# yangao07/abPOA

Measured on NVIDIA B200. Metric: GCUPS (DP cells/s), global/convex 10 kbp, higher is better.
Workload: dtype int16 (packed int16x2 DPX arithmetic; int32 kernel only as overflow fallback)

## Files before the change

abpoa_b200/csrc/poa_kernels.cu:

```cuda
#include <cuda_runtime.h>
#include <stdint.h>
#include <algorithm>
#include "poa_device.cuh"
#include "poa_chain.cuh"

#define FULL 0xffffffffu
#define NEG POA_NEG32

enum { LG = 0, AG = 1, CG = 2 };
enum { GLOBAL = 0, LOCAL = 1, EXTEND = 2 };

#define OP_M   0x1
#define OP_E1  0x2
#define OP_E2  0x4
#define OP_E   0x6
#define OP_F1  0x8
#define OP_F2  0x10
#define OP_F   0x18
#define OP_ALL 0x1f

__device__ __forceinline__ void ld8(const int16_t *p, int v[8]) {
    const uint4 u = *reinterpret_cast<const uint4 *>(p);
    v[0] = (int)(short)(u.x & 0xffff); v[1] = ((int)u.x) >> 16;
    v[2] = (int)(short)(u.y & 0xffff); v[3] = ((int)u.y) >> 16;
// ... 815 lines not shown
        c.KF1[k] = pk_host(-(oe1 + e1 * (2 * k - 1)), -(oe1 + e1 * (2 * k))); c.KF2[k] = pk_host(-(oe2 + e2 * (2 * k - 1)), -(oe2 + e2 * (2 * k)));
        c.KLG[k] = pk_host(-e1 * (2 * k), -e1 * (2 * k + 1));
    }
    c.NE1 = pk_host(-e1, -e1); c.NOE1 = pk_host(-oe1, -oe1); c.NE2 = pk_host(-e2, -e2); c.NOE2 = pk_host(-oe2, -oe2);
    return c;
}

struct P16Smem {
    int *mat_s; uint4 *cap_lo, *cap_hi, *ring_meta; int16_t *ring_data;
};
__device__ __forceinline__ P16Smem p16_smem_init(uint8_t *dyn_smem, const PoaParamsDev *prm, int ring_rows, int lane) {
    P16Smem sm;
    sm.mat_s = reinterpret_cast<int *>(dyn_smem);
    sm.cap_lo = reinterpret_cast<uint4 *>(dyn_smem + POA_MAX_M * POA_MAX_M * sizeof(int));
    sm.cap_hi = sm.cap_lo + 9;
    sm.ring_meta = sm.cap_hi + 9;
    sm.ring_data = reinterpret_cast<int16_t *>(sm.ring_meta + ring_rows);
    const int m = prm->m;
    for (int t = lane; t < m * m; t += 32) sm.mat_s[t] = prm->mat[t];
    if (lane < 9) {
        unsigned lo[4], hi[4];
#pragma unroll
        for (int k = 0; k < 4; ++k) {
            lo[k] = pk(2 * k < lane ? NEGP : 32767, 2 * k + 1 < lane ? NEGP : 32767);
            hi[k] = pk(2 * k >= 8 - lane ? NEGP : 32767, 2 * k + 1 >= 8 - lane ? NEGP : 32767);
        }
        sm.cap_lo[lane] = make_uint4(lo[0], lo[1], lo[2], lo[3]);
        sm.cap_hi[lane] = make_uint4(hi[0], hi[1], hi[2], hi[3]);
    }
    __syncwarp();
    return sm;
}

template <int GAP, int MODE, bool LEAN = false, bool TMA = false>
__device__ __forceinline__ void p16_run_job(const PoaJobDesc &jd, const PoaParamsDev *__restrict__ prm, const P16Consts &kc, const P16Smem &sm,
                                            int ring_rows, int ring_cells, int lane) {
    typedef int16_t ST;
    typedef Planes<GAP> PL;
    constexpr int RN = RingPlanes<GAP>::N;
    int *mat_s = sm.mat_s; uint4 *cap_lo = sm.cap_lo, *cap_hi = sm.cap_hi, *ring_meta = sm.ring_meta; ST *ring_data = sm.ring_data;
    const int rmask = ring_rows - 1, ring_groups = ring_cells >> 3;
    const long long clk0 = clock64();
    uint64_t t_start_ns; asm volatile("mov.u64 %0, %%globaltimer;" : "=l"(t_start_ns));
    const int m = prm->m;
    const JobView jv = open_job(jd.blob);
    ST *planes = reinterpret_cast<ST *>(jd.planes);
    PoaRowInfo *rowinfo = jd.rowinfo; PoaRowOff *rowoff = jd.rowoff;
    const int qlen = jv.qlen, n_rows = jv.n_rows, w = jv.w;
    const bool banded = w >= 0;
    const int e1 = prm->e1, o1 = prm->o1, oe1 = prm->oe1, e2 = prm->e2, o2 = prm->o2, oe2 = prm->oe2;
    const int pnv = jv.pn;
    const unsigned zr2 = (unsigned)prm->zero;

    PoaResultDev res;
    res.status = POA_ST_OK; res.best_score = NEG; res.best_i = 0; res.best_j = 0; res.n_ops = 0;
    res.start_i = res.start_j = 0; res.n_aln_bases = res.n_matched_bases = 0; res.max_band = 0; res.cells = 0; res.plane_units_used = 0;
    res.fwd_clk = 0; res.bt_clk = 0; res.t_start_ns = t_start_ns; res.t_end_ns = 0;

    int16_t *qp = jd.qprof;
    const int qstride = ((qlen + 1 + 7) & ~7) + 8;
    for (int r = 0; r < m; ++r)
        for (int j = lane; j < qstride; j += 32)
            qp[(size_t)r * qstride + j] = (j == 0 || j > qlen) ? (int16_t)0 : (int16_t)mat_s[r * m + jv.qs[j]];
    __syncwarp();

    uint64_t cursor = 0;
    int64_t cells = 0; int max_band = 0;
    int best_score = NEG, best_i = 0, best_j = 0, best_row = 0;
    int guard_lo = 0, guard_hi = 0;
    bool stop = false;

    {
        int end0 = qlen;
        if (banded) end0 = min(qlen, max(0, qlen - jv.remain(0)) + w);
        const int g1 = end0 >> 3, ngrp = g1 + 1;
        if ((uint64_t)ngrp * PL::N > jd.plane_cap_units) { if (lane == 0) { res.status = POA_ST_PLANE_OVF; *jd.result = res; } return; }
        for (int gp = 0; gp <= g1; gp += 32) {
            const int g = gp + lane;
            if (g <= g1) {
                int h[8], ea[8], eb[8], fa[8], fb[8];
#pragma unroll
                for (int c = 0; c < 8; ++c) {
                    const int j = g * 8 + c;
                    if (MODE == LOCAL) { h[c] = ea[c] = eb[c] = fa[c] = fb[c] = (j <= end0) ? 0 : NEGP; }
                    else if (j > end0) { h[c] = ea[c] = eb[c] = fa[c] = fb[c] = NEGP; }
                    else if (GAP == LG) { h[c] = max(-e1 * j, NEGP); }
                    else if (j == 0) { h[c] = 0; ea[c] = -oe1; eb[c] = -oe2; fa[c] = fb[c] = NEGP; }
                    else {
                        fa[c] = max(-o1 - e1 * j, NEGP); fb[c] = max(-o2 - e2 * j, NEGP); ea[c] = eb[c] = NEGP;
                        h[c] = (GAP == CG) ? max(fa[c], fb[c]) : fa[c];
                    }
                }
                ST *rp = planes + (size_t)g * POA_GROUP;
                st8(rp, h);
                if (GAP != LG) { st8(rp + (size_t)PL::E1 * ngrp * POA_GROUP, ea); st8(rp + (size_t)PL::F1 * ngrp * POA_GROUP, fa); }
                if (GAP == CG) { st8(rp + (size_t)PL::E2 * ngrp * POA_GROUP, eb); st8(rp + (size_t)PL::F2 * ngrp * POA_GROUP, fb); }
                if (g < ring_groups) {
                    ST *rq = ring_data + (size_t)g * POA_GROUP;
                    st8(rq, h);
                    if (GAP != LG) st8(rq + ring_cells, ea);
                    if (GAP == CG) st8(rq + 2 * ring_cells, eb);
                }
            }
        }
        if (lane == 0) {
            PoaRowInfo r0; r0.beg = 0; r0.end = end0; r0.left = 0; r0.right = 0;
            rowinfo[0] = r0; { PoaRowOff z; z.off = 0; z.p0 = -1; rowoff[0] = z; } ring_meta[0] = make_uint4(0u, (unsigned)end0, 1u | (1u << 16), 0u);
        }
        cursor = (uint64_t)ngrp * PL::N;
        cells += end0 + 1; max_band = end0 + 1;
        __syncwarp();
    }

    const uint32_t ring_s = (uint32_t)__cvta_generic_to_shared(ring_data);
    constexpr int RS = TMA ? PL::N : RN;
    const uint32_t ring_row_bytes = (uint32_t)(RS * ring_cells * 2), ring_plane_bytes = (uint32_t)(ring_cells * 2);
    const int pn_shift = pnv == 16 ? 4 : 3;
    const uint32_t cap32 = jd.plane_cap_units > 0xffffffffull ? 0xffffffffu : (uint32_t)jd.plane_cap_units;
    uint32_t cur32 = (uint32_t)cursor;
    const bool has_ps = LEAN ? false : (jv.predscore != nullptr);

    const int npred_tot = ldb(&jv.rowmeta[n_rows].x);
    int pb = 0, pe = 0, rbase = 0, rem = 0, raw_pred = -1, raw_ps = 0;
    if (n_rows > 2) {
        { const int2 m1 = ldb(jv.rowmeta + 1); pb = m1.x; pe = jv.predoff(2); rbase = m1.y & 0xff; rem = m1.y >> 8; }
        { const int k = max(min(pb + lane, npred_tot - 1), 0); raw_pred = ldb(jv.pred + k); if (has_ps) raw_ps = ldb(jv.predscore + k); }
    }
    int nx_y = n_rows > 3 ? ldb(&jv.rowmeta[2].y) : 0;
    constexpr int LP = 4;
    int lp_c[LP];
#pragma unroll
    for (int k = 0; k < LP; ++k) lp_c[k] = LEAN ? __shfl_sync(FULL, lane < pe - pb ? raw_pred : -1, k) : -1;
    KP_DECL
    for (int i = 1; i < n_rows - 1 && !stop; ++i) {
        KP(5)
        const int np = pe - pb;
        const int mypred = lane < np ? raw_pred : -1, myps = lane < np ? raw_ps : 0;
        int lp[LP];
#pragma unroll
        for (int k = 0; k < LP; ++k) lp[k] = lp_c[k];
        int2 m2;
        m2.x = ldb(&jv.rowmeta[i + 2].x); m2.y = ldb(&jv.rowmeta[i + 2].y);
        const int n_rbase = nx_y & 0xff, n_rem = nx_y >> 8;
        int n_raw_pred, n_raw_ps = 0;
        { const int k = max(min(pe + lane, npred_tot - 1), 0); n_raw_pred = ldb(jv.pred + k); if (has_ps) n_raw_ps = ldb(jv.predscore + k); }
        if (LEAN || !(jv.live && !ldb(jv.live + i))) {

        bool lean_row = false;
        uint4 lm[LP];
#pragma unroll
        for (int k = 0; k < LP; ++k) lm[k] = make_uint4(0u, 0u, 0u, 0u);
        if (LEAN) {
            lean_row = np >= 1 && np <= LP;
#pragma unroll
            for (int k = 0; k < LP; ++k) if (k < np && (i - lp[k]) > rmask) lean_row = false;
#ifdef POA_KPROF
            if (!lean_row) { if (np > LP || np < 1) ++kdiag[1]; else ++kdiag[2]; }
#endif
            if (lean_row) {
                lm[0] = ring_meta[lp[0] & rmask];
                int wide = (int)(lm[0].y >> 3) - (int)(lm[0].x >> 3) + 1;
#pragma unroll
                for (int k = 1; k < LP; ++k) {
                    lm[k] = k < np ? ring_meta[lp[k] & rmask] : lm[0];
                    wide = max(wide, (int)(lm[k].y >> 3) - (int)(lm[k].x >> 3) + 1);
                }
                if (wide > ring_groups) lean_row = false;
#ifdef POA_KPROF
                if (lean_row) ++kdiag[0]; else ++kdiag[3];
#endif
            }
        }
        unsigned wA = 0, wB = 0;
        int l1 = INT32_MAX, r1 = INT32_MIN, b1 = INT32_MAX;
        if (!lean_row && lane < np) {
            const int prow = mypred;
            const bool near = (i - prow) <= rmask;
            uint4 mi;
            if (near) mi = ring_meta[prow & rmask];
            else { const PoaRowInfo pi = rowinfo[prow]; mi = make_uint4((unsigned)pi.beg, (unsigned)pi.end, (unsigned)(pi.left + 1) | ((unsigned)(pi.right + 1) << 16), rowoff[prow].off); }
            l1 = (int)(mi.z & 0xffffu); r1 = (int)(mi.z >> 16); b1 = (int)mi.x;
            const unsigned pg0 = mi.x >> 3, png = (mi.y >> 3) - pg0 + 1;
            wA = pg0 | (png << 12) | ((unsigned)near << 25) | ((unsigned)(prow & rmask) << 26);
            wB = mi.w;
        }
        int ml = jv.node_n, mr = 0, min_pre_beg = INT32_MAX;
        if (lean_row) {
#pragma unroll
            for (int k = 0; k < LP; ++k) {
                ml = min(ml, (int)(lm[k].z & 0xffffu)); mr = max(mr, (int)(lm[k].z >> 16)); min_pre_beg = min(min_pre_beg, (int)lm[k].x);
            }
        } else if (banded) {
            ml = min(ml, __reduce_min_sync(FULL, l1));
            mr = max(mr, __reduce_max_sync(FULL, r1));
            min_pre_beg = __reduce_min_sync(FULL, b1);
            for (int kb = 32; kb < np; kb += 32) {
                const int k = kb + lane;
                int l2 = INT32_MAX, r2 = INT32_MIN, b2 = INT32_MAX;
                if (k < np) { const PoaRowInfo pi = rowinfo[ldb(jv.pred + pb + k)]; l2 = pi.left + 1; r2 = pi.right + 1; b2 = pi.beg; }
                ml = min(ml, __reduce_min_sync(FULL, l2)); mr = max(mr, __reduce_max_sync(FULL, r2)); min_pre_beg = min(min_pre_beg, __reduce_min_sync(FULL, b2));
            }
        }
        int beg = 0, end = qlen;
        if (banded) {
            const int r = qlen - rem;
            beg = max(0, min(ml, r) - w);
            end = min(qlen, max(mr, r) + w);
            if (np > 0 && (beg >> pn_shift) < (min_pre_beg >> pn_shift)) beg = min_pre_beg;
        }
        const int g0 = beg >> 3, g1 = end >> 3, ngrp = g1 - g0 + 1;
        const uint32_t need = (uint32_t)ngrp * PL::N;
        if (need > cap32 - cur32) {
            if (TMA) { if (lane == 0) asm volatile("cp.async.bulk.wait_group 0;" ::: "memory"); __syncwarp(); }
            if (lane == 0) { res.status = POA_ST_PLANE_OVF; res.plane_units_used = cur32; *jd.result = res; }
            return;
        }
        const bool tma_row = TMA && ngrp <= ring_groups;
        const uint32_t my_off = cur32;
        cur32 += need;
        ST *rowp = planes + (size_t)my_off * POA_GROUP;
        const size_t gplane = (size_t)ngrp * POA_GROUP;
        const uint32_t my_ring_s = ring_s + (uint32_t)(i & rmask) * ring_row_bytes;
        cells += (end >= beg) ? (end - beg + 1) : 0;
        max_band = max(max_band, end - beg + 1);
        const int16_t *qrow = qp + (size_t)rbase * qstride;
        if (i + 1 < n_rows - 1) {
            const int16_t *nrow = qp + (size_t)n_rbase * qstride;
            const int c0 = min((g0 + lane) * 8, qstride - 8);
            asm volatile("prefetch.global.L1 [%0];" :: "l"(nrow + c0));
            if (lane >= 24) asm volatile("prefetch.global.L1 [%0];" :: "l"(nrow + min(c0 + 64, qstride - 8)));
        }

        int carry1 = 2 * NEG, carry2 = 2 * NEG;
        int row_max = NEG, row_left = -1, row_right = -1;
        KP(0)

        for (int gp = g0; gp <= g1; gp += 32) {
            const int g = gp + lane;
            const bool active = g <= g1;
            uint4 sv = make_uint4(0u, 0u, 0u, 0u);
            if (active) sv = *reinterpret_cast<const uint4 *>(qrow + (size_t)g * 8);
            unsigned M[4], X1[4], X2[4];
            unsigned D0[4];
#pragma unroll
            for (int k = 0; k < 4; ++k) { M[k] = NEGP2; X1[k] = NEGP2; X2[k] = NEGP2; D0[k] = NEGP2; }
            const bool fix_left = (gp > g0) || ((beg & 7) == 0);

            if (lean_row) {
#pragma unroll
                for (int k = 0; k < LP; ++k) {
                    if (k >= np) break;
                    const uint4 mi = lm[k];
                    const int pg0 = (int)(mi.x >> 3), png = (int)(mi.y >> 3) - pg0 + 1;
                    const int rel = g - pg0;
                    const bool inr = active && (unsigned)rel < (unsigned)png;
                    const uint32_t prs = ring_s + (uint32_t)(lp[k] & rmask) * ring_row_bytes;
                    uint4 hp = make_uint4(NEGP2, NEGP2, NEGP2, NEGP2), ep1 = hp, ep2 = hp;
                    if (inr) {
                        const uint32_t a = prs + (uint32_t)rel * 16u;
                        asm volatile("ld.shared.v4.u32 {%0,%1,%2,%3}, [%4];" : "=r"(hp.x), "=r"(hp.y), "=r"(hp.z), "=r"(hp.w) : "r"(a));
                        if (GAP != LG) asm volatile("ld.shared.v4.u32 {%0,%1,%2,%3}, [%4];" : "=r"(ep1.x), "=r"(ep1.y), "=r"(ep1.z), "=r"(ep1.w) : "r"(a + ring_plane_bytes));
                        if (GAP == CG) asm volatile("ld.shared.v4.u32 {%0,%1,%2,%3}, [%4];" : "=r"(ep2.x), "=r"(ep2.y), "=r"(ep2.z), "=r"(ep2.w) : "r"(a + 2 * ring_plane_bytes));
                    }
                    unsigned prev = __shfl_up_sync(FULL, hp.w, 1);
                    if (fix_left) {
                        if (lane == 0) {
                            int hm1 = NEGP;
                            const int relm = rel - 1;
                            if ((unsigned)relm < (unsigned)png) { unsigned short v; asm volatile("ld.shared.u16 %0, [%1];" : "=h"(v) : "r"(prs + (uint32_t)relm * 16u + 14u)); hm1 = (int)(short)v; }
// ... 67 lines not shown
                    }
                    unsigned d0 = sh1(prev, hp.x), d1 = sh1(hp.x, hp.y), d2 = sh1(hp.y, hp.z), d3 = sh1(hp.z, hp.w);
                    if (has_ps) {
                        const int ps = __shfl_sync(FULL, c_ps, k);
                        const unsigned ps2 = pk(ps, ps);
                        d0 = __viaddmax_s16x2(d0, ps2, NEGP2); d1 = __viaddmax_s16x2(d1, ps2, NEGP2);
                        d2 = __viaddmax_s16x2(d2, ps2, NEGP2); d3 = __viaddmax_s16x2(d3, ps2, NEGP2);
                        if (GAP == LG) {
                            hp.x = __viaddmax_s16x2(hp.x, ps2, NEGP2); hp.y = __viaddmax_s16x2(hp.y, ps2, NEGP2);
                            hp.z = __viaddmax_s16x2(hp.z, ps2, NEGP2); hp.w = __viaddmax_s16x2(hp.w, ps2, NEGP2);
                        } else {
                            ep1.x = __viaddmax_s16x2(ep1.x, ps2, NEGP2); ep1.y = __viaddmax_s16x2(ep1.y, ps2, NEGP2);
                            ep1.z = __viaddmax_s16x2(ep1.z, ps2, NEGP2); ep1.w = __viaddmax_s16x2(ep1.w, ps2, NEGP2);
                            if (GAP == CG) {
                                ep2.x = __viaddmax_s16x2(ep2.x, ps2, NEGP2); ep2.y = __viaddmax_s16x2(ep2.y, ps2, NEGP2);
                                ep2.z = __viaddmax_s16x2(ep2.z, ps2, NEGP2); ep2.w = __viaddmax_s16x2(ep2.w, ps2, NEGP2);
                            }
                        }
                    }
                    if (kb == 0 && k == 0) { D0[0] = d0; D0[1] = d1; D0[2] = d2; D0[3] = d3; }
                    M[0] = __vmaxs2(M[0], d0); M[1] = __vmaxs2(M[1], d1); M[2] = __vmaxs2(M[2], d2); M[3] = __vmaxs2(M[3], d3);
                    if (GAP == LG) {
                        X1[0] = __vmaxs2(X1[0], __viaddmax_s16x2(hp.x, kc.NE1, NEGP2)); X1[1] = __vmaxs2(X1[1], __viaddmax_s16x2(hp.y, kc.NE1, NEGP2));
                        X1[2] = __vmaxs2(X1[2], __viaddmax_s16x2(hp.z, kc.NE1, NEGP2)); X1[3] = __vmaxs2(X1[3], __viaddmax_s16x2(hp.w, kc.NE1, NEGP2));
                    } else {
                        X1[0] = __vmaxs2(X1[0], ep1.x); X1[1] = __vmaxs2(X1[1], ep1.y); X1[2] = __vmaxs2(X1[2], ep1.z); X1[3] = __vmaxs2(X1[3], ep1.w);
                        if (GAP == CG) { X2[0] = __vmaxs2(X2[0], ep2.x); X2[1] = __vmaxs2(X2[1], ep2.y); X2[2] = __vmaxs2(X2[2], ep2.z); X2[3] = __vmaxs2(X2[3], ep2.w); }
                    }
                }
            }

            KP(1)
            const int nlo = min(max(beg - g * 8, 0), 8), nhi = min(max(g * 8 + 7 - end, 0), 8);
            const uint4 clo = cap_lo[nlo], chi = cap_hi[nhi];
            const unsigned CLO[4] = { clo.x, clo.y, clo.z, clo.w };
            const unsigned CAP[4] = { __vmins2(clo.x, chi.x), __vmins2(clo.y, chi.y), __vmins2(clo.z, chi.z), __vmins2(clo.w, chi.w) };
            const unsigned S[4] = { sv.x, sv.y, sv.z, sv.w };

            unsigned T[4], H[4], F1[4], F2[4], E1o[4], E2o[4];
#pragma unroll
            for (int k = 0; k < 4; ++k) {
                const unsigned hm = __viaddmax_s16x2(M[k], S[k], NEGP2);
                M[k] = __vmins2(hm, CLO[k]);
                if (GAP == LG) T[k] = __vmins2(__vmaxs2(hm, X1[k]), CLO[k]);
                else if (GAP == AG) T[k] = M[k];
                else T[k] = __vmins2(__vimax3_s16x2(hm, X1[k], X2[k]), CLO[k]);
            }
            const int jr0 = (g - g0) * 8;
            unsigned a1[4], a2[4];
#pragma unroll
            for (int k = 0; k < 4; ++k) { a1[k] = __vadd2(T[k], kc.K1[k]); if (GAP == CG) a2[k] = __vadd2(T[k], kc.K2[k]); }
            const int off1 = e1 * jr0 - (GAP == LG ? 0 : oe1), off2 = e2 * jr0 - oe2;
            int tot1, tot2 = 0;
            int x1 = max(warp_excl_max(lane_max8(a1) + off1, lane, tot1), carry1);
            carry1 = max(carry1, tot1);
            const int xl1 = min(max(x1 - off1, NEGP), 32767);
            unsigned P1[4], P2[4];
            lane_excl_prefix(a1, pk(xl1, xl1), P1);
            if (GAP == CG) {
                int x2 = max(warp_excl_max(lane_max8(a2) + off2, lane, tot2), carry2);
                carry2 = max(carry2, tot2);
                const int xl2 = min(max(x2 - off2, NEGP), 32767);
                lane_excl_prefix(a2, pk(xl2, xl2), P2);
            }
#pragma unroll
            for (int k = 0; k < 4; ++k) {
                if (GAP == LG) {
                    unsigned h = __viaddmax_s16x2(__vmaxs2(P1[k], a1[k]), kc.KLG[k], NEGP2);
                    if (MODE == LOCAL) h = __vmaxs2(h, zr2);
                    H[k] = __vmins2(h, CAP[k]);
                } else {
                    F1[k] = __viaddmax_s16x2(P1[k], kc.KF1[k], NEGP2);
                    if (GAP == AG) {
                        const unsigned t = __vmaxs2(M[k], X1[k]);
                        unsigned fz = F1[k];
                        if (MODE == LOCAL) fz = __vmaxs2(fz, zr2);
                        const unsigned h = __vmaxs2(t, fz);
                        const unsigned from_t = __vcmpges2(t, fz);
                        const unsigned ev = __viaddmax_s16x2(X1[k], kc.NE1, __viaddmax_s16x2(h, kc.NOE1, NEGP2));
                        const unsigned alt = (MODE == LOCAL) ? zr2 : NEGP2;
                        E1o[k] = __vmins2((ev & from_t) | (alt & ~from_t), CAP[k]);
                        H[k] = __vmins2(h, CAP[k]);
                    } else {
                        F2[k] = __viaddmax_s16x2(P2[k], kc.KF2[k], NEGP2);
                        unsigned h = __vimax3_s16x2(T[k], F1[k], F2[k]);
                        if (MODE == LOCAL) h = __vmaxs2(h, zr2);
                        unsigned eo1 = __viaddmax_s16x2(X1[k], kc.NE1, __viaddmax_s16x2(h, kc.NOE1, NEGP2));
                        unsigned eo2 = __viaddmax_s16x2(X2[k], kc.NE2, __viaddmax_s16x2(h, kc.NOE2, NEGP2));
                        if (MODE == LOCAL) { eo1 = __vmaxs2(eo1, zr2); eo2 = __vmaxs2(eo2, zr2); }
                        H[k] = __vmins2(h, CAP[k]); E1o[k] = __vmins2(eo1, CAP[k]); E2o[k] = __vmins2(eo2, CAP[k]);
                    }
                }
            }

            if (jd.btrec != nullptr) {
                unsigned t = 0;
#pragma unroll
                for (int k = 0; k < 4; ++k)
                    t |= __vcmpeq2(__viaddmax_s16x2(D0[k], S[k], NEGP2), H[k]) & (0x00020001u << (2 * k));
                const unsigned byte = (t | (t >> 16)) & 0xffu;
                uint8_t *rec = reinterpret_cast<uint8_t *>(jd.btrec + i);
                const int rel = g - g0;
                if (active && rel < POA_BTREC_GROUPS) rec[16 + rel] = (uint8_t)byte;
                if (lane == 0 && gp == g0)
                    *reinterpret_cast<uint4 *>(rec) = make_uint4((unsigned)(g0 * 8), (unsigned)mypred,
                                                                 (unsigned)rbase | (ngrp <= POA_BTREC_GROUPS ? 0x100u : 0u) | ((unsigned)min(ngrp, 0xffff) << 16), (unsigned)my_off);
            }
            KP(2)
            if (TMA && tma_row) {
                if (gp == g0) {
                    if (lane == 0) { if (ring_rows >= 8) asm volatile("cp.async.bulk.wait_group.read 7;" ::: "memory"); else asm volatile("cp.async.bulk.wait_group.read 0;" ::: "memory"); }
                    __syncwarp();
                }
                if (active) {
                    const uint32_t a = my_ring_s + (uint32_t)(g - g0) * 16u;
                    asm volatile("st.shared.v4.u32 [%0], {%1,%2,%3,%4};" :: "r"(a), "r"(H[0]), "r"(H[1]), "r"(H[2]), "r"(H[3]) : "memory");
                    if (GAP != LG) {
                        asm volatile("st.shared.v4.u32 [%0], {%1,%2,%3,%4};" :: "r"(a + (uint32_t)PL::E1 * ring_plane_bytes), "r"(E1o[0]), "r"(E1o[1]), "r"(E1o[2]), "r"(E1o[3]) : "memory");
                        asm volatile("st.shared.v4.u32 [%0], {%1,%2,%3,%4};" :: "r"(a + (uint32_t)PL::F1 * ring_plane_bytes), "r"(F1[0]), "r"(F1[1]), "r"(F1[2]), "r"(F1[3]) : "memory");
                    }
                    if (GAP == CG) {
                        asm volatile("st.shared.v4.u32 [%0], {%1,%2,%3,%4};" :: "r"(a + (uint32_t)PL::E2 * ring_plane_bytes), "r"(E2o[0]), "r"(E2o[1]), "r"(E2o[2]), "r"(E2o[3]) : "memory");
                        asm volatile("st.shared.v4.u32 [%0], {%1,%2,%3,%4};" :: "r"(a + (uint32_t)PL::F2 * ring_plane_bytes), "r"(F2[0]), "r"(F2[1]), "r"(F2[2]), "r"(F2[3]) : "memory");
                    }
                }
            } else
            if (active) {
                const int rel = g - g0;
                if (rel < ring_groups) {
                    const uint32_t a = my_ring_s + (uint32_t)rel * 16u;
                    asm volatile("st.shared.v4.u32 [%0], {%1,%2,%3,%4};" :: "r"(a), "r"(H[0]), "r"(H[1]), "r"(H[2]), "r"(H[3]) : "memory");
                    if (GAP != LG) asm volatile("st.shared.v4.u32 [%0], {%1,%2,%3,%4};" :: "r"(a + ring_plane_bytes), "r"(E1o[0]), "r"(E1o[1]), "r"(E1o[2]), "r"(E1o[3]) : "memory");
                    if (GAP == CG) asm volatile("st.shared.v4.u32 [%0], {%1,%2,%3,%4};" :: "r"(a + 2 * ring_plane_bytes), "r"(E2o[0]), "r"(E2o[1]), "r"(E2o[2]), "r"(E2o[3]) : "memory");
                }
                ST *q = rowp + (size_t)rel * POA_GROUP;
                *reinterpret_cast<uint4 *>(q) = make_uint4(H[0], H[1], H[2], H[3]);
                if (GAP != LG) {
                    *reinterpret_cast<uint4 *>(q + (size_t)PL::E1 * gplane) = make_uint4(E1o[0], E1o[1], E1o[2], E1o[3]);
                    *reinterpret_cast<uint4 *>(q + (size_t)PL::F1 * gplane) = make_uint4(F1[0], F1[1], F1[2], F1[3]);
                }
                if (GAP == CG) {
                    *reinterpret_cast<uint4 *>(q + (size_t)PL::E2 * gplane) = make_uint4(E2o[0], E2o[1], E2o[2], E2o[3]);
                    *reinterpret_cast<uint4 *>(q + (size_t)PL::F2 * gplane) = make_uint4(F2[0], F2[1], F2[2], F2[3]);
                }
            }

            KP(3)
            {
                const int lmax = active ? lane_max8(H) : NEGP;
                unsigned eq = 0;
#pragma unroll
                for (int k = 0; k < 4; ++k) { eq |= (unsigned)(lo16(H[k]) == lmax) << (2 * k); eq |= (unsigned)(hi16(H[k]) == lmax) << (2 * k + 1); }
                const int lfirst = g * 8 + __ffs(eq) - 1, llast = g * 8 + 31 - __clz(eq);
                const int pm = __reduce_max_sync(FULL, lmax);
                const unsigned bm = __ballot_sync(FULL, lmax == pm && pm > NEGP);
                if (bm) {
                    const int pl = __shfl_sync(FULL, lfirst, __ffs(bm) - 1);
                    const int pr = __shfl_sync(FULL, llast, 31 - __clz(bm));
                    if (pm > row_max) { row_max = pm; row_left = pl; row_right = pr; }
                    else if (pm == row_max) row_right = pr;
                }
            }
        }
        KP(4)
        if (TMA && tma_row) {
            asm volatile("fence.proxy.async.shared::cta;" ::: "memory");
            __syncwarp();
            if (lane == 0) {
                const uint32_t bytes = (uint32_t)ngrp * 16u;
#pragma unroll
                for (int pl = 0; pl < PL::N; ++pl)
                    asm volatile("cp.async.bulk.global.shared::cta.bulk_group [%0], [%1], %2;"
                                 :: "l"(rowp + (size_t)pl * gplane), "r"(my_ring_s + (uint32_t)pl * ring_plane_bytes), "r"(bytes) : "memory");
                asm volatile("cp.async.bulk.commit_group;" ::: "memory");
            }
        }
        if (lane == 0) {
            ring_meta[i & rmask] = make_uint4((unsigned)beg, (unsigned)end, (unsigned)(row_left + 1) | ((unsigned)(row_right + 1) << 16), my_off);
            PoaRowInfo ri; ri.beg = beg; ri.end = end; ri.left = row_left; ri.right = row_right;
            rowinfo[i] = ri; { PoaRowOff z; z.off = my_off; z.p0 = mypred; *reinterpret_cast<uint2 *>(rowoff + i) = make_uint2(z.off, (unsigned)z.p0); }
        }
        guard_lo |= (row_max < -14000); guard_hi |= (row_max > 29000);
        if (MODE == LOCAL) {
            if (row_max > best_score) { best_score = row_max; best_i = i; best_j = row_left; }
        } else if (MODE == EXTEND) {
            if (row_max > best_score) { best_score = row_max; best_i = i; best_j = row_right; best_row = i; }
            else if (prm->zdrop > 0) {
                const int delta = jv.remain(best_row) - rem;
                if (best_score - row_max > prm->zdrop + e1 * abs(delta - (row_right - best_j))) stop = true;
            }
        }
        __syncwarp();
        }
        asm volatile("" : "+r"(m2.x), "+r"(m2.y), "+r"(n_raw_pred), "+r"(n_raw_ps));
        pb = pe; pe = m2.x; rbase = n_rbase; rem = n_rem; nx_y = m2.y; raw_pred = n_raw_pred; raw_ps = n_raw_ps;
// ... 151 lines not shown
    const P16Consts kc = make_p16_consts(gaps[0], gaps[1], gaps[2], gaps[3]);
    const bool tma = poa_tma_enabled() && ring_rows >= 2;
    if (gap_mode == LG) return tma ? launch_chain_worker_one<LG, true>(slots, sync, n_groups, prm, ring_rows, ring_cells, kc, st) : launch_chain_worker_one<LG, false>(slots, sync, n_groups, prm, ring_rows, ring_cells, kc, st);
    if (gap_mode == AG) return tma ? launch_chain_worker_one<AG, true>(slots, sync, n_groups, prm, ring_rows, ring_cells, kc, st) : launch_chain_worker_one<AG, false>(slots, sync, n_groups, prm, ring_rows, ring_cells, kc, st);
    return tma ? launch_chain_worker_one<CG, true>(slots, sync, n_groups, prm, ring_rows, ring_cells, kc, st) : launch_chain_worker_one<CG, false>(slots, sync, n_groups, prm, ring_rows, ring_cells, kc, st);
}

template <int GAP, bool TMA>
static cudaError_t launch_chain_one(const PoaChainSlot *slots, const int32_t *idx, int n_jobs, int round, const PoaParamsDev *prm, int ring_rows, int ring_cells,
                                    const P16Consts &kc, cudaStream_t st) {
    const size_t smem = ring_smem_bytes(GAP, 16, ring_rows, ring_cells, TMA) + 18 * sizeof(uint4);
    cudaError_t e = cudaFuncSetAttribute(poa_chain_align_kernel_p16<GAP, TMA>, cudaFuncAttributeMaxDynamicSharedMemorySize, (int)(227 * 1024));
    if (e != cudaSuccess) return e;
    poa_chain_align_kernel_p16<GAP, TMA><<<n_jobs, 32, smem, st>>>(slots, idx, prm, n_jobs, round, ring_rows, ring_cells, kc);
    return cudaGetLastError();
}
extern "C" int poa_tma_enabled(void);
extern "C" cudaError_t poa_launch_chain_align_p16(int gap_mode, const int *gaps, const PoaChainSlot *slots, const int32_t *idx, int n_jobs, int round,
                                                  const PoaParamsDev *prm, int ring_rows, int ring_cells, cudaStream_t st) {
    if (n_jobs <= 0) return cudaSuccess;
    const P16Consts kc = make_p16_consts(gaps[0], gaps[1], gaps[2], gaps[3]);
    if (poa_tma_enabled() && ring_rows >= 2) {
        if (gap_mode == LG) return launch_chain_one<LG, true>(slots, idx, n_jobs, round, prm, ring_rows, ring_cells, kc, st);
        if (gap_mode == AG) return launch_chain_one<AG, true>(slots, idx, n_jobs, round, prm, ring_rows, ring_cells, kc, st);
        return launch_chain_one<CG, true>(slots, idx, n_jobs, round, prm, ring_rows, ring_cells, kc, st);
    }
    if (gap_mode == LG) return launch_chain_one<LG, false>(slots, idx, n_jobs, round, prm, ring_rows, ring_cells, kc, st);
    if (gap_mode == AG) return launch_chain_one<AG, false>(slots, idx, n_jobs, round, prm, ring_rows, ring_cells, kc, st);
    return launch_chain_one<CG, false>(slots, idx, n_jobs, round, prm, ring_rows, ring_cells, kc, st);
}

static inline size_t ring_smem_bytes(int gap, int bits, int ring_rows, int ring_cells, int all_planes) {
    const int rn = all_planes ? (gap == LG ? 1 : (gap == AG ? 3 : 5)) : (gap == LG ? 1 : (gap == AG ? 2 : 3));
    return (size_t)POA_MAX_M * POA_MAX_M * sizeof(int) + (size_t)ring_rows * sizeof(PoaRowInfo) + (((size_t)ring_rows * 4 + 15) & ~(size_t)15)
           + (size_t)ring_rows * rn * ring_cells * (bits / 8);
}

template <int GAP, typename ST, int MODE>
static cudaError_t launch_one(const PoaJobDesc *jobs, const PoaParamsDev *prm, int n_jobs, int ring_rows, int ring_cells, cudaStream_t st) {
    const size_t smem = ring_smem_bytes(GAP, (int)sizeof(ST) * 8, ring_rows, ring_cells);
    cudaError_t e = cudaFuncSetAttribute(poa_align_kernel<GAP, ST, MODE>, cudaFuncAttributeMaxDynamicSharedMemorySize, (int)(227 * 1024));
    if (e != cudaSuccess) return e;
    const char *cv = getenv("ABPOA_GPU_CARVEOUT");
    if (cv && *cv) cudaFuncSetAttribute(poa_align_kernel<GAP, ST, MODE>, cudaFuncAttributePreferredSharedMemoryCarveout, atoi(cv));
    poa_align_kernel<GAP, ST, MODE><<<n_jobs, 32, smem, st>>>(jobs, prm, n_jobs, ring_rows, ring_cells);
    return cudaGetLastError();
}

template <int GAP, typename ST>
static cudaError_t launch_mode(int mode, const PoaJobDesc *jobs, const PoaParamsDev *prm, int n_jobs, int rr, int rc, cudaStream_t st) {
    switch (mode) {
    case GLOBAL: return launch_one<GAP, ST, GLOBAL>(jobs, prm, n_jobs, rr, rc, st);
    case LOCAL:  return launch_one<GAP, ST, LOCAL>(jobs, prm, n_jobs, rr, rc, st);
    default:     return launch_one<GAP, ST, EXTEND>(jobs, prm, n_jobs, rr, rc, st);
    }
}

extern "C" int poa_tma_enabled(void) { static const int on = [] { const char *e = getenv("ABPOA_GPU_TMA"); return e && *e == '1'; }(); return on; }
extern "C" void poa_pick_ring(int gap_mode, int bits, int band_cells, size_t smem_budget, int *ring_rows, int *ring_cells) {
    int rc = band_cells < 64 ? 64 : band_cells;
    int rr = 64;
    const int all = bits == 16 && poa_tma_enabled();
    if (all) smem_budget += 12 * 1024;
    smem_budget = smem_budget > 512 ? smem_budget - 512 : smem_budget;
    while (rr > 2 && ring_smem_bytes(gap_mode, bits, rr, rc, all) > smem_budget) rr >>= 1;
    while (rc > 64 && ring_smem_bytes(gap_mode, bits, rr, rc, all) > smem_budget) rc -= 64;
    *ring_rows = rr; *ring_cells = rc;
}
// ... 46 lines not shown
```

Measured before the change: 126.3.

## Add guard-padded ring rows and single-pass fast predecessor path for narrow int16 rows

Pads each shared-memory ring plane with NEG-filled guard groups on both sides, so predecessor loads for narrow rows can read out of range without bounds checks. A fast path covers rows with at most 32 groups and narrow predecessors: one pass per lane, with predicated vector stores to shared and global memory. The next row's query profile is now loaded into registers ahead of time instead of only prefetched. Cell math and row-max code move into shared helpers, and the guard padding enlarges the shared-memory footprint.

After: 128.1, median of 6. 1.4% higher.

```diff
diff --git a/abpoa_b200/csrc/poa_kernels.cu b/abpoa_b200/csrc/poa_kernels.cu
--- a/abpoa_b200/csrc/poa_kernels.cu
+++ b/abpoa_b200/csrc/poa_kernels.cu
@@ -871,6 +871,141 @@
     return sm;
 }
 
+#define P16_RING_GUARD 2
+#define P16_FAST_GROUPS 32
+__device__ __forceinline__ void sts_v4_if(bool p, uint32_t a, unsigned x, unsigned y, unsigned z, unsigned w) {
+    asm volatile("{ .reg .pred q; setp.ne.b32 q, %0, 0; @q st.shared.v4.u32 [%1], {%2,%3,%4,%5}; }"
+                 :: "r"((int)p), "r"(a), "r"(x), "r"(y), "r"(z), "r"(w) : "memory");
+}
+__device__ __forceinline__ void stg_v4_if(bool p, void *a, const unsigned (&v)[4]) {
+    asm volatile("{ .reg .pred q; setp.ne.b32 q, %0, 0; @q st.global.v4.u32 [%1], {%2,%3,%4,%5}; }"
+                 :: "r"((int)p), "l"(a), "r"(v[0]), "r"(v[1]), "r"(v[2]), "r"(v[3]) : "memory");
+}
+template <int RN>
+__device__ __forceinline__ void p16_ring_guard2(uint32_t a, uint32_t plane_bytes, int lane, int rel, int ring_groups) {
+    const bool p = lane >= 30 && rel + 2 < ring_groups;
+#pragma unroll
+    for (int k = 0; k < RN; ++k) sts_v4_if(p, a + 32u + (uint32_t)k * plane_bytes, NEGP2, NEGP2, NEGP2, NEGP2);
+}
+
+template <int GAP, int NP>
+__device__ __forceinline__ void p16_fast_preds(const uint4 (&lm)[4], const int (&lp)[4], int np, int g, uint32_t ring_s, uint32_t ring_row_bytes,
+                                               uint32_t ring_plane_bytes, int rmask, const P16Consts &kc,
+                                               unsigned (&M)[4], unsigned (&X1)[4], unsigned (&X2)[4], unsigned (&D0)[4]) {
+#pragma unroll
+    for (int k = 0; k < NP; ++k) {
+        const uint4 mi = lm[k];
+        const int prow = k < np ? lp[k] : lp[0];
+        const int pg0 = (int)(mi.x >> 3), png = (int)(mi.y >> 3) - pg0 + 1;
+        const int rel = min(max(g - pg0, -1), png + 1);
+        const uint32_t a = ring_s + (uint32_t)(prow & rmask) * ring_row_bytes + (uint32_t)(rel * 16);
+        uint4 hp, ep1 = make_uint4(0u, 0u, 0u, 0u), ep2 = ep1;
+        unsigned left;
+        asm volatile("ld.shared.v4.u32 {%0,%1,%2,%3}, [%4];" : "=r"(hp.x), "=r"(hp.y), "=r"(hp.z), "=r"(hp.w) : "r"(a));
+        asm volatile("ld.shared.u32 %0, [%1];" : "=r"(left) : "r"(a - 4u));
+        if (GAP != LG) asm volatile("ld.shared.v4.u32 {%0,%1,%2,%3}, [%4];" : "=r"(ep1.x), "=r"(ep1.y), "=r"(ep1.z), "=r"(ep1.w) : "r"(a + ring_plane_bytes));
+        if (GAP == CG) asm volatile("ld.shared.v4.u32 {%0,%1,%2,%3}, [%4];" : "=r"(ep2.x), "=r"(ep2.y), "=r"(ep2.z), "=r"(ep2.w) : "r"(a + 2 * ring_plane_bytes));
+        const unsigned d0 = sh1(left, hp.x), d1 = sh1(hp.x, hp.y), d2 = sh1(hp.y, hp.z), d3 = sh1(hp.z, hp.w);
+        if (GAP == LG) {
+            hp.x = __viaddmax_s16x2(hp.x, kc.NE1, NEGP2); hp.y = __viaddmax_s16x2(hp.y, kc.NE1, NEGP2); hp.z = __viaddmax_s16x2(hp.z, kc.NE1, NEGP2); hp.w = __viaddmax_s16x2(hp.w, kc.NE1, NEGP2);
+        }
+        const uint4 x1 = GAP == LG ? hp : ep1;
+        if (k == 0) {
+            D0[0] = d0; D0[1] = d1; D0[2] = d2; D0[3] = d3;
+            M[0] = d0; M[1] = d1; M[2] = d2; M[3] = d3;
+            X1[0] = x1.x; X1[1] = x1.y; X1[2] = x1.z; X1[3] = x1.w;
+            X2[0] = ep2.x; X2[1] = ep2.y; X2[2] = ep2.z; X2[3] = ep2.w;
+        } else {
+            M[0] = __vmaxs2(M[0], d0); M[1] = __vmaxs2(M[1], d1); M[2] = __vmaxs2(M[2], d2); M[3] = __vmaxs2(M[3], d3);
+            X1[0] = __vmaxs2(X1[0], x1.x); X1[1] = __vmaxs2(X1[1], x1.y); X1[2] = __vmaxs2(X1[2], x1.z); X1[3] = __vmaxs2(X1[3], x1.w);
+            if (GAP == CG) { X2[0] = __vmaxs2(X2[0], ep2.x); X2[1] = __vmaxs2(X2[1], ep2.y); X2[2] = __vmaxs2(X2[2], ep2.z); X2[3] = __vmaxs2(X2[3], ep2.w); }
+        }
+    }
+}
+
+template <int GAP, int MODE>
+__device__ __forceinline__ void p16_cells(const P16Consts &kc, const uint4 clo, const uint4 chi, const uint4 sv, int g, int g0, int lane,
+                                          int e1, int oe1, int e2, int oe2, unsigned zr2, int &carry1, int &carry2,
+                                          unsigned (&M)[4], const unsigned (&X1)[4], const unsigned (&X2)[4],
+                                          unsigned (&H)[4], unsigned (&E1o)[4], unsigned (&E2o)[4], unsigned (&F1)[4], unsigned (&F2)[4]) {
+    const unsigned CLO[4] = { clo.x, clo.y, clo.z, clo.w };
+    const unsigned CAP[4] = { __vmins2(clo.x, chi.x), __vmins2(clo.y, chi.y), __vmins2(clo.z, chi.z), __vmins2(clo.w, chi.w) };
+    const unsigned S[4] = { sv.x, sv.y, sv.z, sv.w };
+    unsigned T[4];
+#pragma unroll
+    for (int k = 0; k < 4; ++k) {
+        const unsigned hm = __viaddmax_s16x2(M[k], S[k], NEGP2);
+        M[k] = __vmins2(hm, CLO[k]);
+        if (GAP == LG) T[k] = __vmins2(__vmaxs2(hm, X1[k]), CLO[k]);
+        else if (GAP == AG) T[k] = M[k];
+        else T[k] = __vmins2(__vimax3_s16x2(hm, X1[k], X2[k]), CLO[k]);
+    }
+    const int jr0 = (g - g0) * 8;
+    unsigned a1[4], a2[4];
+#pragma unroll
+    for (int k = 0; k < 4; ++k) { a1[k] = __vadd2(T[k], kc.K1[k]); if (GAP == CG) a2[k] = __vadd2(T[k], kc.K2[k]); }
+    const int off1 = e1 * jr0 - (GAP == LG ? 0 : oe1), off2 = e2 * jr0 - oe2;
+    int tot1, tot2 = 0;
+    int x1 = max(warp_excl_max(lane_max8(a1) + off1, lane, tot1), carry1);
+    carry1 = max(carry1, tot1);
+    const int xl1 = min(max(x1 - off1, NEGP), 32767);
+    unsigned P1[4], P2[4];
+    lane_excl_prefix(a1, pk(xl1, xl1), P1);
+    if (GAP == CG) {
+        int x2 = max(warp_excl_max(lane_max8(a2) + off2, lane, tot2), carry2);
+        carry2 = max(carry2, tot2);
+        const int xl2 = min(max(x2 - off2, NEGP), 32767);
+        lane_excl_prefix(a2, pk(xl2, xl2), P2);
+    }
+#pragma unroll
+    for (int k = 0; k < 4; ++k) {
+        if (GAP == LG) {
+            unsigned h = __viaddmax_s16x2(__vmaxs2(P1[k], a1[k]), kc.KLG[k], NEGP2);
+            if (MODE == LOCAL) h = __vmaxs2(h, zr2);
+            H[k] = __vmins2(h, CAP[k]);
+        } else {
+            F1[k] = __viaddmax_s16x2(P1[k], kc.KF1[k], NEGP2);
+            if (GAP == AG) {
+                const unsigned t = __vmaxs2(M[k], X1[k]);
+                unsigned fz = F1[k];
+                if (MODE == LOCAL) fz = __vmaxs2(fz, zr2);
+                const unsigned h = __vmaxs2(t, fz);
+                const unsigned from_t = __vcmpges2(t, fz);
+                const unsigned ev = __viaddmax_s16x2(X1[k], kc.NE1, __viaddmax_s16x2(h, kc.NOE1, NEGP2));
+                const unsigned alt = (MODE == LOCAL) ? zr2 : NEGP2;
+                E1o[k] = __vmins2((ev & from_t) | (alt & ~from_t), CAP[k]);
+                H[k] = __vmins2(h, CAP[k]);
+            } else {
+                F2[k] = __viaddmax_s16x2(P2[k], kc.KF2[k], NEGP2);
+                unsigned h = __vimax3_s16x2(T[k], F1[k], F2[k]);
+                if (MODE == LOCAL) h = __vmaxs2(h, zr2);
+                unsigned eo1 = __viaddmax_s16x2(X1[k], kc.NE1, __viaddmax_s16x2(h, kc.NOE1, NEGP2));
+                unsigned eo2 = __viaddmax_s16x2(X2[k], kc.NE2, __viaddmax_s16x2(h, kc.NOE2, NEGP2));
+                if (MODE == LOCAL) { eo1 = __vmaxs2(eo1, zr2); eo2 = __vmaxs2(eo2, zr2); }
+                H[k] = __vmins2(h, CAP[k]); E1o[k] = __vmins2(eo1, CAP[k]); E2o[k] = __vmins2(eo2, CAP[k]);
+            }
+        }
+    }
+}
+
+__device__ __forceinline__ void p16_row_max(const unsigned (&H)[4], bool active, int g, int &row_max, int &row_left, int &row_right) {
+    const int lmax = active ? lane_max8(H) : NEGP;
+    const unsigned lb = pk(lmax, lmax);
+    unsigned t = 0;
+#pragma unroll
+    for (int k = 0; k < 4; ++k) t |= __vcmpeq2(H[k], lb) & (0x00020001u << (2 * k));
+    const unsigned eq = (t | (t >> 16)) & 0xffu;
+    const int lfirst = g * 8 + __ffs(eq) - 1, llast = g * 8 + 31 - __clz(eq);
+    const int pm = __reduce_max_sync(FULL, lmax);
+    const unsigned bm = __ballot_sync(FULL, lmax == pm && pm > NEGP);
+    if (bm) {
+        const int pl = __shfl_sync(FULL, lfirst, __ffs(bm) - 1);
+        const int pr = __shfl_sync(FULL, llast, 31 - __clz(bm));
+        if (pm > row_max) { row_max = pm; row_left = pl; row_right = pr; }
+        else if (pm == row_max) row_right = pr;
+    }
+}
+
 template <int GAP, int MODE, bool LEAN = false, bool TMA = false>
 __device__ __forceinline__ void p16_run_job(const PoaJobDesc &jd, const PoaParamsDev *__restrict__ prm, const P16Consts &kc, const P16Smem &sm,
                                             int ring_rows, int ring_cells, int lane) {
@@ -909,6 +1044,13 @@
     int guard_lo = 0, guard_hi = 0;
     bool stop = false;
 
+    constexpr int RS = TMA ? PL::N : RN;
+    const int ring_plane_cells = ring_cells + P16_RING_GUARD * POA_GROUP;
+    ST *const ring_row0 = ring_data + P16_RING_GUARD * POA_GROUP;
+    for (int t = lane; t < ring_rows * RS * P16_RING_GUARD; t += 32)
+        *reinterpret_cast<uint4 *>(ring_data + (size_t)(t / P16_RING_GUARD) * ring_plane_cells + (t % P16_RING_GUARD) * POA_GROUP) =
+            make_uint4(NEGP2, NEGP2, NEGP2, NEGP2);
+
     {
         int end0 = qlen;
         if (banded) end0 = min(qlen, max(0, qlen - jv.remain(0)) + w);
@@ -935,12 +1077,17 @@
                 if (GAP != LG) { st8(rp + (size_t)PL::E1 * ngrp * POA_GROUP, ea); st8(rp + (size_t)PL::F1 * ngrp * POA_GROUP, fa); }
                 if (GAP == CG) { st8(rp + (size_t)PL::E2 * ngrp * POA_GROUP, eb); st8(rp + (size_t)PL::F2 * ngrp * POA_GROUP, fb); }
                 if (g < ring_groups) {
-                    ST *rq = ring_data + (size_t)g * POA_GROUP;
+                    ST *rq = ring_row0 + (size_t)g * POA_GROUP;
                     st8(rq, h);
-                    if (GAP != LG) st8(rq + ring_cells, ea);
-                    if (GAP == CG) st8(rq + 2 * ring_cells, eb);
-                }
-            }
+                    if (GAP != LG) st8(rq + ring_plane_cells, ea);
+                    if (GAP == CG) st8(rq + 2 * ring_plane_cells, eb);
+                }
+            }
+        }
+        if (lane < 2 && g1 + 1 + lane < ring_groups) {
+            ST *rq = ring_row0 + (size_t)(g1 + 1 + lane) * POA_GROUP;
+#pragma unroll
+            for (int p = 0; p < RN; ++p) *reinterpret_cast<uint4 *>(rq + p * ring_plane_cells) = make_uint4(NEGP2, NEGP2, NEGP2, NEGP2);
         }
         if (lane == 0) {
             PoaRowInfo r0; r0.beg = 0; r0.end = end0; r0.left = 0; r0.right = 0;
@@ -951,9 +1098,8 @@
         __syncwarp();
     }
 
-    const uint32_t ring_s = (uint32_t)__cvta_generic_to_shared(ring_data);
-    constexpr int RS = TMA ? PL::N : RN;
-    const uint32_t ring_row_bytes = (uint32_t)(RS * ring_cells * 2), ring_plane_bytes = (uint32_t)(ring_cells * 2);
+    const uint32_t ring_s = (uint32_t)__cvta_generic_to_shared(ring_row0);
+    const uint32_t ring_row_bytes = (uint32_t)(RS * ring_plane_cells * 2), ring_plane_bytes = (uint32_t)(ring_plane_cells * 2);
     const int pn_shift = pnv == 16 ? 4 : 3;
     const uint32_t cap32 = jd.plane_cap_units > 0xffffffffull ? 0xffffffffu : (uint32_t)jd.plane_cap_units;
     uint32_t cur32 = (uint32_t)cursor;
@@ -966,6 +1112,8 @@
         { const int k = max(min(pb + lane, npred_tot - 1), 0); raw_pred = ldb(jv.pred + k); if (has_ps) raw_ps = ldb(jv.predscore + k); }
     }
     int nx_y = n_rows > 3 ? ldb(&jv.rowmeta[2].y) : 0;
+    int pf_g0 = -2;
+    uint4 pf_a = make_uint4(0u, 0u, 0u, 0u), pf_b = pf_a;
     constexpr int LP = 4;
     int lp_c[LP];
 #pragma unroll
@@ -985,7 +1133,7 @@
         { const int k = max(min(pe + lane, npred_tot - 1), 0); n_raw_pred = ldb(jv.pred + k); if (has_ps) n_raw_ps = ldb(jv.predscore + k); }
         if (LEAN || !(jv.live && !ldb(jv.live + i))) {
 
-        bool lean_row = false;
+        bool lean_row = false, fast_preds = false;
         uint4 lm[LP];
 #pragma unroll
         for (int k = 0; k < LP; ++k) lm[k] = make_uint4(0u, 0u, 0u, 0u);
@@ -1005,6 +1153,7 @@
                     wide = max(wide, (int)(lm[k].y >> 3) - (int)(lm[k].x >> 3) + 1);
                 }
                 if (wide > ring_groups) lean_row = false;
+                fast_preds = !TMA && wide <= min(P16_FAST_GROUPS, ring_groups - 2);
 #ifdef POA_KPROF
                 if (lean_row) ++kdiag[0]; else ++kdiag[3];
 #endif
@@ -1063,10 +1212,14 @@
         cells += (end >= beg) ? (end - beg + 1) : 0;
         max_band = max(max_band, end - beg + 1);
         const int16_t *qrow = qp + (size_t)rbase * qstride;
-        if (i + 1 < n_rows - 1) {
-            const int16_t *nrow = qp + (size_t)n_rbase * qstride;
+        const bool pf_hit = (unsigned)(g0 - pf_g0) <= 1u;
+        const uint4 sv_pf = g0 == pf_g0 ? pf_a : pf_b;
+        {
+            const int16_t *nrow = qp + (size_t)min(n_rbase, m - 1) * qstride;
             const int c0 = min((g0 + lane) * 8, qstride - 8);
-            asm volatile("prefetch.global.L1 [%0];" :: "l"(nrow + c0));
+            pf_a = *reinterpret_cast<const uint4 *>(nrow + c0);
+            pf_b = *reinterpret_cast<const uint4 *>(nrow + min(c0 + 8, qstride - 8));
+            pf_g0 = g0;
             if (lane >= 24) asm volatile("prefetch.global.L1 [%0];" :: "l"(nrow + min(c0 + 64, qstride - 8)));
         }
 
@@ -1074,6 +1227,46 @@
         int row_max = NEG, row_left = -1, row_right = -1;
         KP(0)
 
+        if (fast_preds && ngrp <= 32 && ngrp <= ring_groups) {
+            const int g = g0 + lane;
+            const bool active = lane < ngrp;
+            uint4 sv = sv_pf;
+            if (!pf_hit) sv = *reinterpret_cast<const uint4 *>(qrow + (size_t)min(g, g1) * 8);
+            unsigned M[4], X1[4], X2[4], D0[4];
+            if (np == 1) p16_fast_preds<GAP, 1>(lm, lp, np, g, ring_s, ring_row_bytes, ring_plane_bytes, rmask, kc, M, X1, X2, D0);
+            else if (np == 2) p16_fast_preds<GAP, 2>(lm, lp, np, g, ring_s, ring_row_bytes, ring_plane_bytes, rmask, kc, M, X1, X2, D0);
+            else p16_fast_preds<GAP, LP>(lm, lp, np, g, ring_s, ring_row_bytes, ring_plane_bytes, rmask, kc, M, X1, X2, D0);
+            KP(1)
+            const int nlo = min(max(beg - g * 8, 0), 8), nhi = min(max(g * 8 + 7 - end, 0), 8);
+            unsigned H[4], F1[4], F2[4], E1o[4], E2o[4];
+            p16_cells<GAP, MODE>(kc, cap_lo[nlo], cap_hi[nhi], sv, g, g0, lane, e1, oe1, e2, oe2, zr2, carry1, carry2, M, X1, X2, H, E1o, E2o, F1, F2);
+            if (jd.btrec != nullptr) {
+                const unsigned S[4] = { sv.x, sv.y, sv.z, sv.w };
+                unsigned t = 0;
+#pragma unroll
+                for (int k = 0; k < 4; ++k) t |= __vcmpeq2(__viaddmax_s16x2(D0[k], S[k], NEGP2), H[k]) & (0x00020001u << (2 * k));
+                uint8_t *rec = reinterpret_cast<uint8_t *>(jd.btrec + i);
+                if (active && lane < POA_BTREC_GROUPS) rec[16 + lane] = (uint8_t)((t | (t >> 16)) & 0xffu);
+                if (lane == 0)
+                    *reinterpret_cast<uint4 *>(rec) = make_uint4((unsigned)(g0 * 8), (unsigned)mypred,
+                                                                 (unsigned)rbase | (ngrp <= POA_BTREC_GROUPS ? 0x100u : 0u) | ((unsigned)ngrp << 16), (unsigned)my_off);
+            }
+            KP(2)
+            p16_ring_guard2<RN>(my_ring_s + (uint32_t)lane * 16u, ring_plane_bytes, lane, lane, ring_groups);
+            {
+                const bool in_slot = lane < ring_groups;
+                const uint32_t a = my_ring_s + (uint32_t)lane * 16u;
+                sts_v4_if(in_slot, a, H[0], H[1], H[2], H[3]);
+                if (GAP != LG) sts_v4_if(in_slot, a + ring_plane_bytes, E1o[0], E1o[1], E1o[2], E1o[3]);
+                if (GAP == CG) sts_v4_if(in_slot, a + 2 * ring_plane_bytes, E2o[0], E2o[1], E2o[2], E2o[3]);
+                ST *q = rowp + (size_t)lane * POA_GROUP;
+                stg_v4_if(active, q, H);
+                if (GAP != LG) { stg_v4_if(active, q + (size_t)PL::E1 * gplane, E1o); stg_v4_if(active, q + (size_t)PL::F1 * gplane, F1); }
+                if (GAP == CG) { stg_v4_if(active, q + (size_t)PL::E2 * gplane, E2o); stg_v4_if(active, q + (size_t)PL::F2 * gplane, F2); }
+            }
+            KP(3)
+            p16_row_max(H, active, g, row_max, row_left, row_right);
+        } else
         for (int gp = g0; gp <= g1; gp += 32) {
             const int g = gp + lane;
             const bool active = g <= g1;
@@ -1207,66 +1400,9 @@
 
             KP(1)
             const int nlo = min(max(beg - g * 8, 0), 8), nhi = min(max(g * 8 + 7 - end, 0), 8);
-            const uint4 clo = cap_lo[nlo], chi = cap_hi[nhi];
-            const unsigned CLO[4] = { clo.x, clo.y, clo.z, clo.w };
-            const unsigned CAP[4] = { __vmins2(clo.x, chi.x), __vmins2(clo.y, chi.y), __vmins2(clo.z, chi.z), __vmins2(clo.w, chi.w) };
             const unsigned S[4] = { sv.x, sv.y, sv.z, sv.w };
-
-            unsigned T[4], H[4], F1[4], F2[4], E1o[4], E2o[4];
-#pragma unroll
-            for (int k = 0; k < 4; ++k) {
-                const unsigned hm = __viaddmax_s16x2(M[k], S[k], NEGP2);
-                M[k] = __vmins2(hm, CLO[k]);
-                if (GAP == LG) T[k] = __vmins2(__vmaxs2(hm, X1[k]), CLO[k]);
-                else if (GAP == AG) T[k] = M[k];
-                else T[k] = __vmins2(__vimax3_s16x2(hm, X1[k], X2[k]), CLO[k]);
-            }
-            const int jr0 = (g - g0) * 8;
-            unsigned a1[4], a2[4];
-#pragma unroll
-            for (int k = 0; k < 4; ++k) { a1[k] = __vadd2(T[k], kc.K1[k]); if (GAP == CG) a2[k] = __vadd2(T[k], kc.K2[k]); }
-            const int off1 = e1 * jr0 - (GAP == LG ? 0 : oe1), off2 = e2 * jr0 - oe2;
-            int tot1, tot2 = 0;
-            int x1 = max(warp_excl_max(lane_max8(a1) + off1, lane, tot1), carry1);
-            carry1 = max(carry1, tot1);
-            const int xl1 = min(max(x1 - off1, NEGP), 32767);
-            unsigned P1[4], P2[4];
-            lane_excl_prefix(a1, pk(xl1, xl1), P1);
-            if (GAP == CG) {
-                int x2 = max(warp_excl_max(lane_max8(a2) + off2, lane, tot2), carry2);
-                carry2 = max(carry2, tot2);
-                const int xl2 = min(max(x2 - off2, NEGP), 32767);
-                lane_excl_prefix(a2, pk(xl2, xl2), P2);
-            }
-#pragma unroll
-            for (int k = 0; k < 4; ++k) {
-                if (GAP == LG) {
-                    unsigned h = __viaddmax_s16x2(__vmaxs2(P1[k], a1[k]), kc.KLG[k], NEGP2);
-                    if (MODE == LOCAL) h = __vmaxs2(h, zr2);
-                    H[k] = __vmins2(h, CAP[k]);
-                } else {
-                    F1[k] = __viaddmax_s16x2(P1[k], kc.KF1[k], NEGP2);
-                    if (GAP == AG) {
-                        const unsigned t = __vmaxs2(M[k], X1[k]);
-                        unsigned fz = F1[k];
-                        if (MODE == LOCAL) fz = __vmaxs2(fz, zr2);
-                        const unsigned h = __vmaxs2(t, fz);
-                        const unsigned from_t = __vcmpges2(t, fz);
-                        const unsigned ev = __viaddmax_s16x2(X1[k], kc.NE1, __viaddmax_s16x2(h, kc.NOE1, NEGP2));
-                        const unsigned alt = (MODE == LOCAL) ? zr2 : NEGP2;
-                        E1o[k] = __vmins2((ev & from_t) | (alt & ~from_t), CAP[k]);
-                        H[k] = __vmins2(h, CAP[k]);
-                    } else {
-                        F2[k] = __viaddmax_s16x2(P2[k], kc.KF2[k], NEGP2);
-                        unsigned h = __vimax3_s16x2(T[k], F1[k], F2[k]);
-                        if (MODE == LOCAL) h = __vmaxs2(h, zr2);
-                        unsigned eo1 = __viaddmax_s16x2(X1[k], kc.NE1, __viaddmax_s16x2(h, kc.NOE1, NEGP2));
-                        unsigned eo2 = __viaddmax_s16x2(X2[k], kc.NE2, __viaddmax_s16x2(h, kc.NOE2, NEGP2));
-                        if (MODE == LOCAL) { eo1 = __vmaxs2(eo1, zr2); eo2 = __vmaxs2(eo2, zr2); }
-                        H[k] = __vmins2(h, CAP[k]); E1o[k] = __vmins2(eo1, CAP[k]); E2o[k] = __vmins2(eo2, CAP[k]);
-                    }
-                }
-            }
+            unsigned H[4], F1[4], F2[4], E1o[4], E2o[4];
+            p16_cells<GAP, MODE>(kc, cap_lo[nlo], cap_hi[nhi], sv, g, g0, lane, e1, oe1, e2, oe2, zr2, carry1, carry2, M, X1, X2, H, E1o, E2o, F1, F2);
 
             if (jd.btrec != nullptr) {
                 unsigned t = 0;
@@ -1299,43 +1435,31 @@
                         asm volatile("st.shared.v4.u32 [%0], {%1,%2,%3,%4};" :: "r"(a + (uint32_t)PL::F2 * ring_plane_bytes), "r"(F2[0]), "r"(F2[1]), "r"(F2[2]), "r"(F2[3]) : "memory");
                     }
                 }
-            } else
-            if (active) {
+            } else {
                 const int rel = g - g0;
+                p16_ring_guard2<RN>(my_ring_s + (uint32_t)rel * 16u, ring_plane_bytes, lane, rel, ring_groups);
                 if (rel < ring_groups) {
                     const uint32_t a = my_ring_s + (uint32_t)rel * 16u;
                     asm volatile("st.shared.v4.u32 [%0], {%1,%2,%3,%4};" :: "r"(a), "r"(H[0]), "r"(H[1]), "r"(H[2]), "r"(H[3]) : "memory");
                     if (GAP != LG) asm volatile("st.shared.v4.u32 [%0], {%1,%2,%3,%4};" :: "r"(a + ring_plane_bytes), "r"(E1o[0]), "r"(E1o[1]), "r"(E1o[2]), "r"(E1o[3]) : "memory");
                     if (GAP == CG) asm volatile("st.shared.v4.u32 [%0], {%1,%2,%3,%4};" :: "r"(a + 2 * ring_plane_bytes), "r"(E2o[0]), "r"(E2o[1]), "r"(E2o[2]), "r"(E2o[3]) : "memory");
                 }
-                ST *q = rowp + (size_t)rel * POA_GROUP;
-                *reinterpret_cast<uint4 *>(q) = make_uint4(H[0], H[1], H[2], H[3]);
-                if (GAP != LG) {
-                    *reinterpret_cast<uint4 *>(q + (size_t)PL::E1 * gplane) = make_uint4(E1o[0], E1o[1], E1o[2], E1o[3]);
-                    *reinterpret_cast<uint4 *>(q + (size_t)PL::F1 * gplane) = make_uint4(F1[0], F1[1], F1[2], F1[3]);
-                }
-                if (GAP == CG) {
-                    *reinterpret_cast<uint4 *>(q + (size_t)PL::E2 * gplane) = make_uint4(E2o[0], E2o[1], E2o[2], E2o[3]);
-                    *reinterpret_cast<uint4 *>(q + (size_t)PL::F2 * gplane) = make_uint4(F2[0], F2[1], F2[2], F2[3]);
+                if (active) {
+                    ST *q = rowp + (size_t)rel * POA_GROUP;
+                    *reinterpret_cast<uint4 *>(q) = make_uint4(H[0], H[1], H[2], H[3]);
+                    if (GAP != LG) {
+                        *reinterpret_cast<uint4 *>(q + (size_t)PL::E1 * gplane) = make_uint4(E1o[0], E1o[1], E1o[2], E1o[3]);
+                        *reinterpret_cast<uint4 *>(q + (size_t)PL::F1 * gplane) = make_uint4(F1[0], F1[1], F1[2], F1[3]);
+                    }
+                    if (GAP == CG) {
+                        *reinterpret_cast<uint4 *>(q + (size_t)PL::E2 * gplane) = make_uint4(E2o[0], E2o[1], E2o[2], E2o[3]);
+                        *reinterpret_cast<uint4 *>(q + (size_t)PL::F2 * gplane) = make_uint4(F2[0], F2[1], F2[2], F2[3]);
+                    }
                 }
             }
 
             KP(3)
-            {
-                const int lmax = active ? lane_max8(H) : NEGP;
-                unsigned eq = 0;
-#pragma unroll
-                for (int k = 0; k < 4; ++k) { eq |= (unsigned)(lo16(H[k]) == lmax) << (2 * k); eq |= (unsigned)(hi16(H[k]) == lmax) << (2 * k + 1); }
-                const int lfirst = g * 8 + __ffs(eq) - 1, llast = g * 8 + 31 - __clz(eq);
-                const int pm = __reduce_max_sync(FULL, lmax);
-                const unsigned bm = __ballot_sync(FULL, lmax == pm && pm > NEGP);
-                if (bm) {
-                    const int pl = __shfl_sync(FULL, lfirst, __ffs(bm) - 1);
-                    const int pr = __shfl_sync(FULL, llast, 31 - __clz(bm));
-                    if (pm > row_max) { row_max = pm; row_left = pl; row_right = pr; }
-                    else if (pm == row_max) row_right = pr;
-                }
-            }
+            p16_row_max(H, active, g, row_max, row_left, row_right);
         }
         KP(4)
         if (TMA && tma_row) {
@@ -1553,8 +1677,9 @@
 
 static inline size_t ring_smem_bytes(int gap, int bits, int ring_rows, int ring_cells, int all_planes) {
     const int rn = all_planes ? (gap == LG ? 1 : (gap == AG ? 3 : 5)) : (gap == LG ? 1 : (gap == AG ? 2 : 3));
+    const int plane_cells = ring_cells + (bits == 16 ? P16_RING_GUARD * POA_GROUP : 0);
     return (size_t)POA_MAX_M * POA_MAX_M * sizeof(int) + (size_t)ring_rows * sizeof(PoaRowInfo) + (((size_t)ring_rows * 4 + 15) & ~(size_t)15)
-           + (size_t)ring_rows * rn * ring_cells * (bits / 8);
+           + (size_t)ring_rows * rn * plane_cells * (bits / 8);
 }
 
 template <int GAP, typename ST, int MODE>
```
